# pr0g/ToyMeshPathTracer

Measured on AMD Instinct MI355X. Metric: MRays/s on sponza.obj 1920x1080 64spp at 1/2/4/8 GPUs; %HBM roofline, higher is better.
Workload: dtype f32

## Files before the change

toymeshpathtracer_amd/csrc/tmpt_api.cpp:

```cpp
#include <dlfcn.h>
#include <hip/hip_runtime.h>
#include <rccl/rccl.h>
#include <string.h>

#include <algorithm>
#include <new>
#include <chrono>
#include <string>
#include <thread>
#include <vector>

#include "tmpt.h"
#include "tmpt_internal.h"
#include "tmpt_traverse.h"
#include "tmpt_render.h"
#include "tmpt_query_key.h"

namespace tmpt {

static thread_local std::string g_last_error;
void set_error(const std::string& msg) { g_last_error = msg; }
const char* last_error() { return g_last_error.c_str(); }

int load_obj(const char* path, std::vector<float>& tris, f3& bmin, f3& bmax);
// ... 79 lines not shown
    {"sah_c_leaf", true, 0, 1e6, nullptr, &Options::sah_c_leaf, nullptr},
    {"sah_c_tri", true, 0, 1e6, nullptr, &Options::sah_c_tri, nullptr},
    {"sample_base", false, 0, 64512, &Options::sample_base, nullptr, nullptr},
    {"sample_block", false, 0, 1024, &Options::sample_block, nullptr, nullptr},
    {"sample_tail", false, -1, 64, &Options::sample_tail, nullptr, nullptr},
    {"sbuf_max", false, 0, 1e18, nullptr, nullptr, &Options::sbuf_max},
    {"sbuf_pair", false, 0, 1, &Options::sbuf_pair, nullptr, nullptr},
    {"cam_pre", false, -1, 1, &Options::cam_pre, nullptr, nullptr},
    {"cam_pre_max", false, 0, 1e18, nullptr, nullptr, &Options::cam_pre_max},
    {"shadow_split", false, 0, 1, &Options::shadow_split, nullptr, nullptr},
    {"shadow_split_max", false, 0, 1e18, nullptr, nullptr, &Options::shadow_split_max},
    {"shadow_split_pass", false, 0, 1024, &Options::shadow_split_pass, nullptr, nullptr},
    {"pilot", false, -1, 512, &Options::pilot, nullptr, nullptr},
    {"help", false, -1, 1, &Options::help, nullptr, nullptr},
    {"pair", false, -1, 63, &Options::pair, nullptr, nullptr},
    {"balance", false, 0, 1, &Options::balance, nullptr, nullptr},
    {"dprio", false, 0, 1, &Options::dprio, nullptr, nullptr},
    {"wave_cap", false, 0, 64, &Options::wave_cap, nullptr, nullptr},
    {"pixel_chains", false, -1, 1024, &Options::pixel_chains, nullptr, nullptr},
    {"tie_defer", false, -1, 1, &Options::tie_defer, nullptr, nullptr},
    {"redo_cap", false, 0, 1 << 30, &Options::redo_cap, nullptr, nullptr},
    {"redo_inline", false, 0, 1, &Options::redo_inline, nullptr, nullptr},
    {"redo_lanes", false, 1, 64, &Options::redo_lanes, nullptr, nullptr},
    {"path_waves", false, 0, 6, &Options::path_waves, nullptr, nullptr},
    {"top_walk", false, -1, 8, &Options::top_walk, nullptr, nullptr},
    {"shadow_order", false, -1, 2, &Options::shadow_order, nullptr, nullptr},
    {"pop_cull", false, -1, 1, &Options::pop_cull, nullptr, nullptr},
    {"pop_key_cap", false, -1, kPopKeyMax, &Options::pop_key_cap, nullptr, nullptr},
    {"rowspec", false, 0, 1, &Options::rowspec, nullptr, nullptr},
    {"rowspec_wmax", false, 0, 16384, &Options::rowspec_wmax, nullptr, nullptr},
    {"rowspec_windows", false, 0, 32, &Options::rowspec_windows, nullptr, nullptr},
    {"rowspec_spread", false, -1, 100, nullptr, &Options::rowspec_spread, nullptr},
    {"rowspec_groups", false, 1, kRowSpecMaxGroups, &Options::rowspec_groups, nullptr, nullptr},
    {"rowspec_noshadow", false, 0, 1, &Options::rowspec_noshadow, nullptr, nullptr},
    {"rowspec_chase", false, 0, 1, &Options::rowspec_chase, nullptr, nullptr},
    {"rowspec_stream", false, 0, 1, &Options::rowspec_stream, nullptr, nullptr},
    {"rowstream_dynamic", false, 0, 1, &Options::rowstream_dynamic, nullptr, nullptr},
    {"row_flag_leaves", false, 0, 1, &Options::row_flag_leaves, nullptr, nullptr},
    {"row_occ", false, 0, 5, &Options::row_occ, nullptr, nullptr},
    {"wf_bins", false, 1, 8, &Options::wf_bins, nullptr, nullptr},
    {"rowstream_test_abort", false, 0, 1, &Options::rowstream_test_abort, nullptr, nullptr},
    {"tie_rule", false, 0, 1, &Options::tie_rule, nullptr, nullptr},
    {"aov_group", false, 0, 16, &Options::aov_group, nullptr, nullptr},
    {"octree_build", false, 0, 1, &Options::octree_build, nullptr, nullptr},
    {"octree_dev_max", false, 0, 1e18, nullptr, nullptr, &Options::octree_dev_max},
    {"denoise_lds", false, -1, 1, &Options::denoise_lds, nullptr, nullptr},
// ... 266 lines not shown
    if (s.stream.ensure(hipStreamNonBlocking) != hipSuccess) return fail((set_error("tmpt_scene_create: no stream"), -1));
    DeviceBuffer<float> d_tris;
    if (n > 0) {
        if (!d_tris.alloc(sizeof(float) * 9 * (size_t)n))
            return fail((set_error("tmpt_scene_create: out of device memory"), -1));
        if (hipMemcpy(d_tris, tris, sizeof(float) * 9 * (size_t)n, hipMemcpyHostToDevice) != hipSuccess)
            return fail((set_error("tmpt_scene_create: upload failed"), -1));
    }
    s.tris_host.assign(tris, tris + 9 * (size_t)n);
    const int rc = build_lbvh(s.bvh, s.opt, s.stream, d_tris);
    d_tris.reset();
    if (rc) return fail(rc);
    *out = h;
    return 0;
    TMPT_GUARD_END
}

int tmpt_scene_destroy(tmpt_scene* h)
{
    if (!h) return 0;
    Scene& s = h->s;
    (void)hipSetDevice(s.device);
    if (s.stream) (void)hipStreamSynchronize(s.stream);
    for (auto& st : s.rs_stream)
        if (st) (void)hipStreamSynchronize(st);
    delete h;
    return 0;
}

int tmpt_scene_build_octree(tmpt_scene* h, const float bmin[3], const float bmax[3])
{
    TMPT_GUARD_BEGIN
    if (!h || !bmin || !bmax) return bad("tmpt_scene_build_octree: null argument");
    Scene& s = h->s;
    if ((int64_t)s.tris_host.size() != 9 * (int64_t)s.bvh.n) return bad("tmpt_scene_build_octree: no triangle copy");
    TMPT_HIP(hipSetDevice(s.device));
    const auto t0 = std::chrono::steady_clock::now();
    OctreeHost t;
    Octree o;
    const bool on_device = s.opt.octree_build == 1;
    double wmax[3] = {0.0, 0.0, 0.0};
    if (on_device) {
        (void)hipGetLastError();
        if (int rc = build_octree_device(s, bmin, bmax, o, wmax)) return rc;
    } else {
        build_octree(s.tris_host.data(), s.bvh.n, bmin, bmax, t);
// ... 243 lines not shown
    }
    return rc;
    TMPT_GUARD_END
}

int tmpt_scene_get_option(const tmpt_scene* h, const char* key, double* value)
{
    TMPT_GUARD_BEGIN
    if (!h || !value) return bad("tmpt_scene_get_option: null argument");
    if (key && strcmp(key, "pop_key_bits") == 0) {
        *value = (double)pop_key_bits(h->s.bvh.link_bits, h->s.opt.pop_key_cap);
        return 0;
    }
    if (key && strcmp(key, "cam_rays_used") == 0) {
        *value = (double)h->s.cam_rays_used;
        return 0;
    }
    if (key && strcmp(key, "shadow_split_used") == 0) {
        *value = (double)h->s.split_used;
        return 0;
    }
    if (key && strcmp(key, "path_waves_used") == 0) {
        *value = (double)h->s.path_waves_used;
        return 0;
    }
    if (key && strcmp(key, "shadow_split_resolve_ms") == 0) {
        *value = h->s.split_resolve_ms;
        return 0;
    }
    if (key && strcmp(key, "update_kind") == 0) {
        *value = (double)h->s.update_kind;
        return 0;
    }
    if (key && strcmp(key, "update_ms") == 0) {
        *value = h->s.update_ms;
        return 0;
    }
    if (key && strcmp(key, "live_device_objects") == 0) {
        *value = (double)g_live_device_objects.load();
        return 0;
    }
    if (key && strcmp(key, "query_ms") == 0) return (*value = h->s.query_ms, 0);
    if (key && strcmp(key, "query_sort_ms") == 0) return (*value = h->s.query_sort_ms, 0);
    if (key && strcmp(key, "query_chunks") == 0) return (*value = (double)h->s.query_chunks, 0);
    if (key && strcmp(key, "query_sorted") == 0) return (*value = (double)h->s.query_sorted, 0);
    if (key && strcmp(key, "bvh_cost") == 0) {
// ... 1016 lines not shown
```

toymeshpathtracer_amd/csrc/tmpt_device.h:

```cpp
#pragma once

#include <hip/hip_runtime.h>
#include <stdint.h>

#include <atomic>
#include <utility>

namespace tmpt {

inline std::atomic<int64_t> g_live_device_objects{0};

inline size_t free_budget(size_t num, size_t den, size_t already_held)
{
    size_t fr = 0, tot = 0;
    if (hipMemGetInfo(&fr, &tot) != hipSuccess) fr = 0;
    return fr / den * num + already_held;
}

template <typename T = void>
class DeviceBuffer {
public:
    DeviceBuffer() = default;
    DeviceBuffer(DeviceBuffer&& o) noexcept : p_(std::exchange(o.p_, nullptr)), bytes_(std::exchange(o.bytes_, 0)) {}
    DeviceBuffer& operator=(DeviceBuffer&& o) noexcept
// ... 111 lines not shown
    Stream(Stream&& o) noexcept : h_(std::exchange(o.h_, nullptr)) {}
    ~Stream() { reset(); }
    hipStream_t get() const { return h_; }
    operator hipStream_t() const { return h_; }
    void reset()
    {
        if (h_) {
            (void)hipStreamDestroy(h_);
            --g_live_device_objects;
        }
        h_ = nullptr;
    }
    hipError_t ensure(unsigned flags = hipStreamNonBlocking)
    {
        if (h_) return hipSuccess;
        const hipError_t e = hipStreamCreateWithFlags(&h_, flags);
        if (e != hipSuccess) {
            h_ = nullptr;
            return e;
        }
        ++g_live_device_objects;
        return hipSuccess;
    }

private:
    hipStream_t h_ = nullptr;
};

}
```

toymeshpathtracer_amd/csrc/tmpt_internal.h:

```cpp
#pragma once

#include <hip/hip_runtime.h>
#include <stdint.h>

#include <string>
#include <vector>

#include "tmpt_device.h"
#include "tmpt_math.h"

namespace tmpt {

struct alignas(16) Bvh4Node {
    float4 a;
    uint4 b;
    uint4 c;
    int4 d;
};
static_assert(sizeof(Bvh4Node) == 64, "BVH4Q node is one half cache line");

constexpr int kLeafMaxTris = 16;

constexpr int kPopKeyMin = 9;
constexpr int kPopKeyMax = 16;
// ... 195 lines not shown
    int pilot = -1;
    int help = -1;
    int pair = -1;
    int balance = 1;
    int dprio = 1;
    int wave_cap = 0;
    int pixel_chains = -1;
    int rowspec = 1;
    int rowspec_wmax = 0;
    int rowspec_windows = 0;
    float rowspec_spread = -1.0f;
    int rowspec_groups = 2;
    int rowspec_noshadow = 1;
    int rowspec_chase = 1;
    int rowspec_stream = 1;
    int rowstream_test_abort = 0;
    int wf_bins = 1;
    int tie_rule = 0;
    int tie_defer = -1;
    int redo_cap = 0;
    int redo_lanes = 4;
    int path_waves = 0;
    int redo_inline = 1;
    int top_walk = -1;
    int shadow_order = -1;
    int pop_cull = -1;
    int pop_key_cap = -1;
    int aov_group = 0;
    int motion_tile = -1;
    int octree_build = 0;
    double octree_dev_max = 0.0;
    int query_sort = -1;
    int query_top = -1;
    double query_max = 0.0;
    int query_chunk = 1 << 22;
    int query_grid = 0;
    int query_legacy = 0;
    int denoise_lds = -1;
};
int options_parse(Options& o, const char* text, bool allow_build);
int options_set(Options& o, const char* key, double value, bool allow_build);
int options_get(const Options& o, const char* key, double* value);

struct Bvh {
    int32_t n = 0;
    int32_t n_nodes = 0;
// ... 7 lines not shown
    SoaScene soa;
    std::vector<int32_t> level_begin;
    DeviceBuffer<float> node_box;
    DeviceBuffer<float> rec_box;
    double build_ms = 0.0;
};

struct Octree {
    DeviceBuffer<OctNode> oct;
    DeviceBuffer<int32_t> oct_refs;
    DeviceBuffer<OctView> oct_view;
    int32_t n_oct = 0, oct_leaves = 0, oct_depth = 0;
    int32_t oct_flat = 0;
    OctGrid oct_grid{};
    int64_t n_oct_refs = 0;
    double oct_build_ms = 0.0;
    float oct_lo[3] = {0, 0, 0}, oct_hi[3] = {0, 0, 0};
};

struct Scene {
    int device = 0;
    Stream stream;
    Stream rs_stream[kRowSpecMaxGroups];
    Bvh bvh;
    std::vector<float> tris_host;
    int32_t update_kind = 0;
    double update_ms = 0.0;
    double cost = 0.0;
    bool cost_known = false;
    Event update_ev[2];
    Octree octree;
    std::vector<DeviceBuffer<>> oct_scratch;
    DeviceBuffer<uint32_t> oct_flags;
    unsigned long long* ties = nullptr;
    uint64_t tie_queries = 0, root_misses = 0, crack_queries = 0;
    int32_t row_engine = 0, stream_fallbacks = 0;
    int64_t chain_pixels = 0;
    Options opt;
    Event wait_ev;
    DeviceBuffer<unsigned long long> counters;
    PinnedBuffer<unsigned long long> counters_host;
    DeviceBuffer<uint32_t> chk;
    Event render_ev[2];
    DeviceBuffer<> ws;
    DeviceBuffer<float> motion_prev;
    DeviceBuffer<> clip_stage;
// ... 3 lines not shown
    DeviceBuffer<uint32_t> jt;
    int32_t jt_spp = 0;
    DeviceBuffer<float4> sbuf;
    DeviceBuffer<> cam_rays;
    int32_t cam_rays_used = 0;
    DeviceBuffer<> split_buf;
    int32_t split_used = 0, split_passes = 0;
    int32_t path_waves_used = 0;
    DeviceBuffer<float4> split_carry;
    bool split_sub = false;
    struct SplitAcc {
        double extend_ms = 0.0, shadow_ms = 0.0, resolve_ms = 0.0, redo_ms = 0.0;
        int64_t redo_samples = 0, redo_late = 0;
        int32_t redo_launches = 0, launches = 0, used = 0;
    } split_acc;
    Event split_ev[3];
    double split_resolve_ms = 0.0;
    DeviceBuffer<uint2> redo;
    uint32_t redo_cap = 0;
    DeviceBuffer<float4> redo_state;
    int64_t redo_samples = 0;
    int64_t redo_late = 0;
    int32_t redo_launches = 0;
    int32_t tie_path = 0;
    bool row_render = false;
    bool pixel_render = false;
    double redo_ms = 0.0;
    uint64_t redo_rays = 0;
    DeviceBuffer<uint32_t> jt2;
    int32_t jt2_n = 0;
    DeviceBuffer<> rs_buf;
    Event rs_event[kRowSpecMaxGroups + 1];
    PinnedBuffer<uint32_t> rs_host;
    DeviceBuffer<> rs_list;
    DeviceBuffer<> rss_buf;
    DeviceBuffer<uint32_t> rss_tab;
    PinnedBuffer<uint32_t> rss_host;
    bool adapt_on = false;
    const uint32_t* adapt_list = nullptr;
    int64_t adapt_n = 0;
    DeviceBuffer<> adapt_buf;
    PinnedBuffer<uint32_t> adapt_host;
    DeviceBuffer<> query_buf;
    Event query_ev[2];
    std::vector<Event> query_sort_ev;
    double query_ms = 0.0, query_sort_ms = 0.0;
// ... 53 lines not shown
```

toymeshpathtracer_amd/csrc/tmpt_path.h:

```cpp
#pragma once

#include "tmpt_render.h"

namespace tmpt {

#ifndef TMPT_RSS_T
#define TMPT_RSS_T 8
#endif
constexpr int kRssT = TMPT_RSS_T;
static_assert(kRssT >= 4 && kRssT <= 31, "the worker's pick key holds the slot in 5 bits");
constexpr uint32_t kRssM24 = 0xFFFFFFu;
struct RsStream {
    unsigned long long* __restrict__ slots;
    unsigned long long* __restrict__ res;
    unsigned long long* __restrict__ chainpos;
    uint32_t* __restrict__ list;
    uint32_t* __restrict__ rowrays;
    uint32_t* __restrict__ lo;
    uint32_t* __restrict__ ctl;
    const uint32_t* __restrict__ anchors;
    const uint32_t* __restrict__ t1;
    const uint32_t* __restrict__ t2;
    uint32_t na, R, rmask;
    uint32_t jlimit;
// ... 124 lines not shown
constexpr int path_tail(int samp) { return samp <= 1 ? kSparse : 2; }

using PathFn = void (*)(SceneView, RenderArgs, PathCtl, uint32_t*, uint32_t*, unsigned long long*);

PathFn path_kernel(const PathVariant& v);
int find_path_kernel(const PathVariant& v, const char* who, PathFn& fn);

struct PixelChains {
    const uint32_t* cpix;
    const float4* cinit;
    int n, smp0, cspp;
};

uint32_t top_walk_cap(const Options& o, int seeding);
uint32_t oct_shadow_check(const Scene& s);

void launch_resolve_px(hipStream_t stream, const float4* sbuf, int64_t P, int32_t spp, float spp_recip,
                       uint32_t* out);

size_t shadow_ovf_words(int device);
int launch_shadow(hipStream_t stream, int device, const SceneView& sv, const uint4* sq, const uint32_t* count,
                  uint32_t cap, uint32_t* head, float4* srec, uint32_t n_rec, uint32_t* ovf);
void launch_split_resolve(hipStream_t stream, const float4* srec, int64_t P, int32_t cnt, float spp_recip,
                          uint32_t* out, const float4* carry_in = nullptr, float4* carry_out = nullptr);

#ifdef TMPT_EXP_WAVETIME
constexpr int kWaveTimeMax = 16384;
bool wavetime_get(unsigned long long* w);
bool rowtime_get(unsigned long long* r, unsigned long long* cl);
void wavetime_put(const unsigned long long* w);
void rowtime_put(const unsigned long long* r);
#endif

}
```

toymeshpathtracer_amd/csrc/tmpt_render.hip:

```cpp
#include <hip/hip_runtime.h>

#include <stdio.h>
#include <stdlib.h>
#include <string.h>

#include <algorithm>
#include <chrono>
#include <cmath>
#include <string>
#include <utility>
#include <vector>

#include "tmpt_lane_path.h"
#include "tmpt_path.h"

namespace tmpt {

#ifdef TMPT_EXP_WAVETIME
__device__ unsigned long long g_wavetime[3 * kWaveTimeMax];
__device__ unsigned long long g_rowtime[kWaveTimeMax];
__device__ unsigned long long g_claimtime[kWaveTimeMax];
bool wavetime_get(unsigned long long* w)
{
    return hipMemcpyFromSymbol(w, HIP_SYMBOL(g_wavetime), 3 * kWaveTimeMax * 8) == hipSuccess;
// ... 92 lines not shown
    const float h[8] = {o.x, o.y, o.z, __uint_as_float(rng), d.x, d.y, d.z, 0.0f};
#pragma unroll
    for (int i = 0; i < 7; ++i) __hip_atomic_store(&w[i], h[i], __ATOMIC_RELAXED, __HIP_MEMORY_SCOPE_AGENT);
    for (uint32_t i = 0; i < depth; ++i)
        __hip_atomic_store(&w[8 + i], light[i * ls], __ATOMIC_RELAXED, __HIP_MEMORY_SCOPE_AGENT);
}

__device__ __forceinline__ void split_rec_put(float4* rec, f3 end, uint32_t depth, const float* light, uint32_t ls)
{
    typedef float f32x4 __attribute__((ext_vector_type(4)));
    f32x4* q = reinterpret_cast<f32x4*>(rec);
    __builtin_nontemporal_store((f32x4){end.x, end.y, end.z, __uint_as_float(depth)}, q);
    if (depth > 0u)
        __builtin_nontemporal_store((f32x4){light[0], light[ls], light[2 * ls], light[3 * ls]}, q + 1);
    if (depth > 4u)
        __builtin_nontemporal_store((f32x4){light[4 * ls], light[5 * ls], light[6 * ls], light[7 * ls]}, q + 2);
    if (depth > 8u) __builtin_nontemporal_store((f32x4){light[8 * ls], light[9 * ls], 0.0f, 0.0f}, q + 3);
}

template <int BLOCK, int SL>
__device__ __forceinline__ void redo_sample(const SceneView& sv, const RenderArgs& a, uint32_t pix, uint32_t smp_depth,
                                            const float4* __restrict__ ps, float4* __restrict__ sbuf, uint32_t sb_ss,
                                            uint32_t sb_sp, uint32_t& rays_e, uint32_t& rays_s,
                                            TravStack<BLOCK, SL>& st, float* lbuf, float4* __restrict__ srec = nullptr)
{
    const uint32_t smp = smp_depth & 0xFFFFu, depth = smp_depth >> 16;
    const float* w = reinterpret_cast<const float*>(ps);
    float h[7];
#pragma unroll
    for (int i = 0; i < 7; ++i) h[i] = __hip_atomic_load(&w[i], __ATOMIC_RELAXED, __HIP_MEMORY_SCOPE_AGENT);
    for (uint32_t i = 0; i < depth; ++i)
        lbuf[i * BLOCK] = __hip_atomic_load(&w[8 + i], __ATOMIC_RELAXED, __HIP_MEMORY_SCOPE_AGENT);
    uint32_t rng = __float_as_uint(h[3]);
    TravCount cnt;
    if (srec) {
        int end_depth = 0;
        const f3 e = trace_path<false, BLOCK, SL, true, false>(sv, mk(h[0], h[1], h[2]), mk(h[4], h[5], h[6]), rng,
                                                               rays_e, rays_s, st, lbuf, cnt, false, (int)depth,
                                                               &end_depth);
        const uint32_t cnt_smp = (uint32_t)(a.smp_end - a.smp_begin);
        split_rec_put(srec + 4 * ((size_t)pix * cnt_smp + (smp - (uint32_t)a.smp_begin)), e, (uint32_t)end_depth, lbuf,
                      BLOCK);
        return;
    }
    const f3 c = trace_path<false, BLOCK, SL, true, false>(sv, mk(h[0], h[1], h[2]), mk(h[4], h[5], h[6]), rng, rays_e,
                                                           rays_s, st, lbuf, cnt, false, (int)depth);
    typedef float f32x4 __attribute__((ext_vector_type(4)));
    __builtin_nontemporal_store((f32x4){c.x, c.y, c.z, 0.0f},
                                reinterpret_cast<f32x4*>(sbuf + ((size_t)smp * sb_ss + (size_t)pix * sb_sp)));
}

__device__ __forceinline__ uint2 redo_load(const uint2* p)
{
    const unsigned long long w =
        __hip_atomic_load(reinterpret_cast<const unsigned long long*>(p), __ATOMIC_RELAXED, __HIP_MEMORY_SCOPE_AGENT);
    return make_uint2((uint32_t)w, (uint32_t)(w >> 32));
}

__device__ __forceinline__ void redo_put(uint2* p, uint32_t pix, uint32_t smp_depth)
{
    __hip_atomic_store(reinterpret_cast<unsigned long long*>(p), ((unsigned long long)smp_depth << 32) | pix,
                       __ATOMIC_RELAXED, __HIP_MEMORY_SCOPE_AGENT);
}

__device__ __forceinline__ void redo_mark(uint2* p)
// ... 5 lines not shown
__global__ void __launch_bounds__(BLOCK) k_redo(SceneView sv, RenderArgs a, uint2* __restrict__ list, uint32_t cap,
                                                const float4* __restrict__ state, float4* __restrict__ sbuf,
                                                uint32_t sb_ss, uint32_t sb_sp,
                                                uint32_t* __restrict__ ovf, unsigned long long* __restrict__ counters)
{
    __shared__ uint32_t s_stack[SL * BLOCK];
    __shared__ float s_light[kMaxDepth * BLOCK];
    __shared__ uint4 s_top[kTopNodes * 4];
    const int64_t gtid = (int64_t)blockIdx.x * BLOCK + threadIdx.x;
    TravStack<BLOCK, SL> st{&s_stack[threadIdx.x], ovf + gtid * (kStackTotal - SL)};
    const uint32_t ntop = (uint32_t)min(kTopNodes, sv.n_nodes4);
    const uint4* g = reinterpret_cast<const uint4*>(sv.nodes4);
    for (uint32_t i = threadIdx.x; i < ntop * 4; i += BLOCK) s_top[i] = g[i];
    __syncthreads();
    st.top = (const lds_u4*)s_top;
    st.ntop = ntop;
    const uint32_t n = (uint32_t)min(counters[kRedoCounter], (unsigned long long)cap);
    uint32_t rays_e = 0, rays_s = 0;
    for (uint32_t i = (uint32_t)gtid; i < n; i += gridDim.x * BLOCK) {
        const uint2 e = list[i];
        if (e.x >= kRedoDone) continue;
        redo_sample<BLOCK, SL>(sv, a, e.x, e.y, state + (size_t)i * kRedoState4, sbuf, sb_ss, sb_sp, rays_e, rays_s,
                               st, &s_light[threadIdx.x], SPLIT ? sbuf : nullptr);
    }
    const uint32_t re = wave_sum(rays_e), rs = wave_sum(rays_s);
    if (lane_id() == 0 && re + rs) {
        atomicAdd(&counters[0], (unsigned long long)(re + rs));
        atomicAdd(&counters[3], (unsigned long long)re);
        atomicAdd(&counters[kRedoRaysCounter], (unsigned long long)(re + rs));
    }
}

static void free_redo(Scene& s)
{
    s.redo.reset();
    s.redo_state.reset();
    s.redo_cap = 0;
}
static bool alloc_redo(Scene& s, int64_t cap)
{
    free_redo(s);
    if (!s.redo.alloc(sizeof(uint2) * (size_t)cap) ||
        !s.redo_state.alloc(sizeof(float4) * kRedoState4 * (size_t)cap)) {
        free_redo(s);
        return false;
    }
// ... 463 lines not shown
                            settled = true;
                        }
                    } while (T != 0);
                }
            }
            bool finish = false, want_off = false, emit = false;
            f3 color = mk(0.0f, 0.0f, 0.0f);
            if (has_pix && !in_query && !cam) {
                if (HELP && waiting) {
                    finish = true;
                    if (depth < (uint32_t)kMaxDepth) color = sky(r.d);
                } else if (!qany) {
                    bool drop = false;
                    if (DEFER) {
                        drop = octree_flag(sv, r, ts);
                        if (wany(drop)) {
                            if (drop) {
                                const unsigned long long slot = atomicAdd(&counters[kRedoCounter], 1ull);
                                if (slot < (unsigned long long)pc.redo_cap) {
                                    redo_state_put(pc.redo_state + (size_t)slot * kRedoState4, r.o, r.d, rng, light,
                                                   depth, LS);
                                    __builtin_amdgcn_fence(__ATOMIC_RELEASE, "agent");
                                    redo_put(pc.redo + slot, pix, smp | (depth << 16));
                                }
                                rays_e -= 1u;
                                depth = 0;
                                ts.best = -1;
                            }
                        }
                        ts.best >>= 1;
                    } else if (SAMP >= 2) {
                        const bool tie = octree_flag(sv, r, ts);
                        if (wany(tie)) {
                            if (tie) settle_closest<BLOCK, SL, true, SOA, false>(sv, r, 0.0f, kMinT, kMaxT, ts, st);
                        }
                        if (!tie) ts.best >>= 1;
                    } else if (!settled) {
                        ts.best >>= 1;
                    }
                    if (ts.best >= 0) {
                        const float4* hp = reinterpret_cast<const float4*>(sv.tri_orig + ts.best);
                        float4 ha = hp[0], hb = hp[1], hc = hp[2];
                        f3 rnd = random_unit_vector(rng);
                        materialize(ha, hb, hc);
                        const f3 nrm = mk(hc.y, hc.z, hc.w);
                        const f3 pos = hit_pos(mk(ha.x, ha.y, ha.z), mk(ha.w, hb.x, hb.y), mk(hb.z, hb.w, hc.x),
// ... 1071 lines not shown
        int64_t nb = std::min<int64_t>(P, tail_blocks * grid * kBlk);
        while (nb > 0 && (P - nb) + nb * (int64_t)blk >= (1ll << 31)) nb /= 2;
        if (nb > 0) {
            ua = (uint32_t)(P - nb);
            P = (P - nb) + nb * (int64_t)blk;
        }
    }
    int pilot = 2 * P <= 5 * (int64_t)grid * kBlk ? 2 : 4;
    if (o.pilot >= 0) pilot = o.pilot;
    const bool ordered = pilot > 0 && !count && !a.jt && a.smp_begin == 0 && a.smp_end == a.spp &&
                         a.spp >= 2 * pilot && P < (1ll << 31);
    const int64_t lanes = (int64_t)grid * kBlk;
    int help = ordered && !prof && 2 * P <= 9 * lanes ? 1 : 0;
    if (o.help >= 0) help = o.help != 0 && !count && !prof && !jt;
    const uint32_t oct_shadow = oct_shadow_check(s);
    if (oct_shadow) help = 0;
    int pair = help && ordered ? (2 * P <= 3 * lanes ? 52 : 56) : 0;
    if (o.pair >= 0) pair = o.pair;
    const bool w5 = jt ? waves5 : waves5p;
    size_t ovf_words = std::max({(size_t)grid4 * (kStackTotal - kPathSL),
                                 (size_t)std::max(grid4, grid5) * (kStackTotal - kPathSL5),
                                 (size_t)grid6 * (kStackTotal - kPathSL6)}) * kBlk;
    if (jt && o.shadow_split != 0) ovf_words = std::max(ovf_words, shadow_ovf_words(s.device));
    const size_t head_words = (size_t)kSeg * kCtr;
    const size_t hist_words = ordered ? radix_sort_hist_words((int32_t)P) : 0;
    const size_t reg_words = ordered ? 2 * (size_t)kSimdKeys + 64 + (size_t)P : 0;
    const size_t extra_words = ordered ? (size_t)P * (4 + 5) + hist_words + reg_words : 0;
    if (ensure_ws(s, (ovf_words + head_words + extra_words) * 4)) return -1;
    uint32_t* heads = s.ws.as<uint32_t>() + ovf_words;
    TMPT_HIP(hipMemsetAsync(heads, 0, head_words * 4, s.stream));
    PathCtl pc;
    memset(&pc, 0, sizeof(pc));
    pc.heads = heads;
    pc.oct_shadow = oct_shadow;
    pc.top_walk = top_walk_cap(o, a.jt ? 0 : 1);
    pc.P = P;
    pc.nblk = nblk;
    pc.blk = blk;
    pc.div_nblk = fastdiv_make(nblk);
    pc.div_blk = fastdiv_make(blk);
    pc.blk0 = blk0;
    pc.ua = ua;
    if (list) pc.order = s.adapt_list;
    RenderArgs as = a;
    if (a.jt) {
        as.bmask = nblk > 1 ? blk - 1u : 2047u;
// ... 70 lines not shown
                PathFn fn6;
                if (int rc = find_path_kernel(v6, "tmpt_render", fn6)) return rc;
                if (occupancy_blocks((const void*)fn6, kBlk, 0) >= 6) {
                    v_main = v6;
                    fn_main = fn6;
                    grid_main = occupancy_grid((const void*)fn6, kBlk, 0, s.device);
                    return 0;
                }
            }
            v_main.sl = w5 ? kPathSL5 : kPathSL;
            v_main.occ = w5 ? 5 : prof ? 1 : 4;
            if (int rc = find_path_kernel(v_main, "tmpt_render", fn_main)) return rc;
            grid_main = occupancy_grid((const void*)fn_main, kBlk, 0, s.device);
            return 0;
        };
        if (int rc = pick_main()) return rc;
        if ((size_t)grid_main * kBlk * (kStackTotal - v_main.sl) > ovf_words) {
            set_error("tmpt_render: internal: stack spill area sized for fewer lanes");
            return -1;
        }
        s.path_waves_used = v_main.occ;
        s.tie_path = !oct ? 0 : redo ? 2 : redo_nomem ? 3 : 1;
        s.path_launches = 1;
        for (int attempt = 0;; ++attempt) {
            pc.redo = redo ? s.redo : nullptr;
            pc.redo_state = redo ? s.redo_state : nullptr;
            pc.redo_cap = redo ? s.redo_cap : 0u;
            pc.redo_inline = o.redo_inline ? 1u : 0u;
            pc.redo_lanes = (uint32_t)std::max(1, std::min(64, o.redo_lanes));
            if (redo) TMPT_HIP(hipMemsetAsync(s.redo, 0xFF, sizeof(uint2) * (size_t)s.redo_cap, s.stream));
            TMPT_HIP(hipEventRecord(s.path_ev[2], s.stream));
            fn_main<<<grid_main, kBlk, 0, s.stream>>>(view(s), as, pc, d_out, s.ws.as<uint32_t>(), d_counters);
            TMPT_HIP(hipGetLastError());
            TMPT_HIP(hipEventRecord(s.path_ev[3], s.stream));
            if (!redo) break;
            TMPT_HIP(hipMemcpyAsync(s.counters_host + kRedoCounter, d_counters + kRedoCounter,
                                    4 * sizeof(unsigned long long), hipMemcpyDeviceToHost, s.stream));
            TMPT_HIP(hipStreamSynchronize(s.stream));
            const unsigned long long n = s.counters_host[kRedoCounter];
            const unsigned long long traced = s.counters_host[kRedoTraced];
            s.redo_samples = (int64_t)n;
            if (n > s.redo_cap && attempt == 0) {
                if (!(n < (1ull << 31) && alloc_redo(s, (int64_t)n))) {
                    redo = false;
                    v_main.ties = 2;
                    if (int rc = pick_main()) return rc;
                    if ((size_t)grid_main * kBlk * (kStackTotal - v_main.sl) > ovf_words) {
                        set_error("tmpt_render: internal: stack spill area sized for fewer lanes");
                        return -1;
                    }
                    s.path_waves_used = v_main.occ;
                    s.redo_samples = 0;
                    s.tie_path = 3;
                }
                TMPT_HIP(hipMemsetAsync(d_counters, 0, kRenderCounters * sizeof(unsigned long long), s.stream));
                TMPT_HIP(hipMemsetAsync(heads, 0, head_words * 4, s.stream));
                if (split_on) TMPT_HIP(hipMemsetAsync(pc.sq_ctl, 0, kSplitCtlWords * 4, s.stream));
                continue;
            }
            s.redo_late = (int64_t)(std::min<unsigned long long>(n, s.redo_cap) - std::min(traced, n));
            if (traced < std::min<unsigned long long>(n, s.redo_cap)) {
                TMPT_HIP(hipEventRecord(s.path_ev[0], s.stream));
                if (split_on)
                    k_redo<kBlk, kPathSL, true><<<grid, kBlk, 0, s.stream>>>(view(s), as, s.redo, s.redo_cap,
                                                                            s.redo_state, pc.srec, pc.sb_ss, pc.sb_sp,
                                                                            s.ws.as<uint32_t>(), d_counters);
                else
                    k_redo<kBlk, kPathSL><<<grid, kBlk, 0, s.stream>>>(view(s), as, s.redo, s.redo_cap, s.redo_state,
                                                                      pc.sbuf, pc.sb_ss, pc.sb_sp, s.ws.as<uint32_t>(),
                                                                      d_counters);
                TMPT_HIP(hipGetLastError());
                TMPT_HIP(hipEventRecord(s.path_ev[1], s.stream));
                s.redo_launches = 1;
            }
            break;
        }
        if (split_on) {
            TMPT_HIP(hipEventRecord(s.split_ev[0], s.stream));
            if (launch_shadow(s.stream, s.device, view(s), pc.sq, pc.sq_ctl, pc.sq_cap, pc.sq_ctl + kCtr, pc.srec,
                              (uint32_t)cam_n, s.ws.as<uint32_t>())) {
                set_error("tmpt_render: k_shadow launch failed");
                return -1;
            }
            TMPT_HIP(hipEventRecord(s.split_ev[1], s.stream));
            launch_split_resolve(s.stream, pc.srec, a.slots, (int32_t)(s1 - s0), a.out_recip, d_out,
                                 a.smp_begin > 0 ? a.prog : nullptr, a.prog);
            TMPT_HIP(hipGetLastError());
            TMPT_HIP(hipEventRecord(s.split_ev[2], s.stream));
            return 0;
        }
        if (pc.sbuf && !s.adapt_on) {
            k_resolve_px<<<(unsigned)((a.slots + 63) / 64), 64, 0, s.stream>>>(
                pc.sbuf, a.slots, a.spp, a.out_recip, d_out, a.smp_begin, a.smp_end, a.prog);
            TMPT_HIP(hipGetLastError());
        }
        return 0;
    }
    s.tie_path = oct ? 1 : 0;
    PathFn fn;
    if (int rc = find_path_kernel(variant(w5, help, flag ? 2 : 0, false), "tmpt_render", fn)) return rc;
    const int grid_px = occupancy_grid((const void*)fn, kBlk, 0, s.device);
    s.path_waves_used = w5 ? 5 : prof ? 1 : 4;
    if ((size_t)grid_px * kBlk * (kStackTotal - (waves5p ? kPathSL5 : kPathSL)) > ovf_words) {
        set_error("tmpt_render: internal: stack spill area sized for fewer lanes");
        return -1;
    }
    uint32_t* base = heads + head_words;
    float4* state = reinterpret_cast<float4*>(base);
    uint32_t* cost = base + 4 * (size_t)P;
    uint32_t* keys = cost + P;
    uint32_t* vals = keys + P;
    uint32_t* tkeys = vals + P;
    uint32_t* tvals = tkeys + P;
// ... 153 lines not shown
    }
    return inside ? 0 : 1;
}

void reset_render_stats(Scene& s)
{
    s.extend_ms = s.shadow_ms = 0;
    s.extend_rays = s.shadow_rays = s.node_visits = s.tri_tests = 0;
    s.shadow_node_visits = s.shadow_tri_tests = 0;
    s.extend_launches = s.shadow_launches = s.iterations = 0;
    s.row_engine = 0;
    s.stream_fallbacks = 0;
    s.chain_pixels = 0;
    s.redo_samples = 0;
    s.redo_late = 0;
    s.redo_launches = 0;
    s.redo_ms = 0.0;
    s.redo_rays = 0;
    s.tie_path = 0;
    s.cam_rays_used = 0;
    s.split_used = 0;
    s.split_passes = 0;
    s.path_waves_used = 0;
    s.split_resolve_ms = 0.0;
}

int camera_rays(Scene& s, const tmpt_camera* cam, const tmpt_render_desc* d, uint32_t* out)
{
    RenderArgs a = make_args(cam, d);
    if (int rc = ensure_sample_tables(s, a.spp, "tmpt_camera_rays")) return rc;
    a.jt = s.jt;
    a.root_check = camera_root_check(s, a.cam);
    const uint32_t cnt = (uint32_t)(a.smp_end - a.smp_begin);
    const int64_t n = a.slots * (int64_t)cnt;
    if (n <= 0) return 0;
    DeviceBuffer<CamRay> buf;
    if (!buf.alloc(sizeof(CamRay) * (size_t)n)) {
        set_error("tmpt_camera_rays: out of device memory");
        return -12;
    }
    launch_cam_rays(s, a, buf);
    hipError_t e = hipGetLastError();
    if (e == hipSuccess) e = hipStreamSynchronize(s.stream);
    if (e == hipSuccess) e = hipMemcpy(out, buf, sizeof(CamRay) * (size_t)n, hipMemcpyDeviceToHost);
    if (e != hipSuccess) {
        set_error(std::string("tmpt_camera_rays: ") + hipGetErrorString(e));
// ... 54 lines not shown
                               unsigned long long* d_counters)
{
    TMPT_ALLOC(s.split_carry.reserve(sizeof(float4) * (size_t)a.slots), "tmpt_render: the shadow split's carried sums");
    Scene::SplitAcc acc;
    int rc = 0;
    int32_t tie_path = 0, passes = 0;
    for (int32_t b = 0; b < a.spp && rc == 0; b += cs, ++passes) {
        RenderArgs ap = a;
        ap.smp_begin = b;
        ap.smp_end = std::min(b + cs, a.spp);
        ap.prog = s.split_carry;
        if (b > 0) {
            TMPT_HIP(hipMemsetAsync(d_counters + kRedoCounter, 0, 4 * sizeof(unsigned long long), s.stream));
            reset_render_stats(s);
        }
        s.split_sub = true;
        rc = render_persistent(s, ap, d_out, false, d_counters);
        s.split_sub = false;
        if (rc) break;
        TMPT_HIP(hipStreamSynchronize(s.stream));
        float k = 0.0f;
        (void)hipEventElapsedTime(&k, s.path_ev[2], s.path_ev[3]);
        acc.extend_ms += k;
        if (s.redo_launches) {
            (void)hipEventElapsedTime(&k, s.path_ev[0], s.path_ev[1]);
            acc.redo_ms += k;
        }
        if (s.split_used) {
            (void)hipEventElapsedTime(&k, s.split_ev[0], s.split_ev[1]);
            acc.shadow_ms += k;
            (void)hipEventElapsedTime(&k, s.split_ev[1], s.split_ev[2]);
            acc.resolve_ms += k;
        }
        acc.redo_samples += s.redo_samples;
        acc.redo_late += s.redo_late;
        acc.redo_launches += s.redo_launches;
        acc.launches += s.path_launches;
        acc.used += s.split_used;
        if (b == 0) tie_path = s.tie_path;
    }
    if (rc) return rc;
    s.split_acc = acc;
    s.split_passes = passes;
    s.tie_path = tie_path;
    return 0;
}

// ... 116 lines not shown
                    ml.push_back((w[3 * i + 1] - t0) * 0.01);
                    ex.push_back((w[3 * i + 2] - t0) * 0.01);
                }
            auto pct = [](std::vector<double> v, double q) {
                if (v.empty()) return 0.0;
                std::sort(v.begin(), v.end());
                return v[std::min(v.size() - 1, (size_t)(q * (v.size() - 1)))];
            };
            fprintf(stderr, "waves %zu; start us p0/p50/p100 %.0f/%.0f/%.0f; main loop end p0/p10/p50/p90/p100 "
                            "%.0f/%.0f/%.0f/%.0f/%.0f; exit p0/p50/p99/p100 %.0f/%.0f/%.0f/%.0f\n",
                    st.size(), pct(st, 0), pct(st, 0.5), pct(st, 1), pct(ml, 0), pct(ml, 0.1), pct(ml, 0.5),
                    pct(ml, 0.9), pct(ml, 1), pct(ex, 0), pct(ex, 0.5), pct(ex, 0.99), pct(ex, 1));
            std::fill(w.begin(), w.end(), 0ull);
            wavetime_put(w.data());
        }
    }
#endif
    if (progressive) s.prog_key[6] = a.smp_end < a.spp ? a.smp_end : -1;
    if (persistent) {
        float k1 = 0.0f, k0 = 0.0f;
        (void)hipEventElapsedTime(&k1, s.path_ev[2], s.path_ev[3]);
        if (s.path_launches == 2) (void)hipEventElapsedTime(&k0, s.path_ev[0], s.path_ev[1]);
        s.extend_ms = (double)k0 + (double)k1;
        if (s.redo_launches) {
            float kr = 0.0f;
            (void)hipEventElapsedTime(&kr, s.path_ev[0], s.path_ev[1]);
            s.redo_ms = kr;
            s.redo_rays = c[kRedoRaysCounter];
        }
        if (s.split_passes > 1) {
            const Scene::SplitAcc& acc = s.split_acc;
            s.extend_ms = acc.extend_ms;
            s.shadow_ms = acc.shadow_ms;
            s.split_resolve_ms = acc.resolve_ms;
            s.redo_ms = acc.redo_ms;
            s.redo_samples = acc.redo_samples;
            s.redo_late = acc.redo_late;
            s.redo_launches = acc.redo_launches;
            s.redo_rays = c[kRedoRaysCounter];
            s.path_launches = acc.launches;
            s.shadow_launches = s.split_used = acc.used;
        } else if (s.split_used) {
            float ks = 0.0f, kr = 0.0f;
            (void)hipEventElapsedTime(&ks, s.split_ev[0], s.split_ev[1]);
            (void)hipEventElapsedTime(&kr, s.split_ev[1], s.split_ev[2]);
            s.shadow_ms = ks;
            s.split_resolve_ms = kr;
// ... 88 lines not shown
```

toymeshpathtracer_amd/csrc/tmpt_shadow.hip:

```cpp
#include "tmpt_path.h"

namespace tmpt {

#ifndef TMPT_SHADOW_SL
#define TMPT_SHADOW_SL 12
#endif
#ifndef TMPT_SHADOW_OCC
#define TMPT_SHADOW_OCC 8
#endif
#ifndef TMPT_SHADOW_STEPS
#define TMPT_SHADOW_STEPS 1
#endif
#ifndef TMPT_SHADOW_FILL
#define TMPT_SHADOW_FILL 16
#endif
constexpr int kShadowSL = TMPT_SHADOW_SL;
constexpr int kShadowOcc = TMPT_SHADOW_OCC;
constexpr int kShadowSteps = TMPT_SHADOW_STEPS;
constexpr int kShadowFillMin = TMPT_SHADOW_FILL;
constexpr uint32_t kShadowFetch = 512u;

template <int BLOCK, int SL>
__global__ void __launch_bounds__(BLOCK, kShadowOcc) k_shadow(SceneView sv, const uint4* __restrict__ sq,
                                                              const uint32_t* __restrict__ count, uint32_t cap,
// ... 78 lines not shown
            if (done) {
                in_query = false;
                if (ts.best >= 0) srec[(size_t)(dst >> 4) * 16u + 4u + (dst & 15u)] = 0.0f;
            }
        }
    }
}

static int shadow_grid(int device)
{
    return occupancy_grid((const void*)k_shadow<kBlk, kShadowSL>, kBlk, 0, device);
}

size_t shadow_ovf_words(int device) { return (size_t)shadow_grid(device) * kBlk * (kStackTotal - kShadowSL); }

int launch_shadow(hipStream_t stream, int device, const SceneView& sv, const uint4* sq, const uint32_t* count,
                  uint32_t cap, uint32_t* head, float4* srec, uint32_t n_rec, uint32_t* ovf)
{
    k_shadow<kBlk, kShadowSL><<<shadow_grid(device), kBlk, 0, stream>>>(sv, sq, count, cap, head,
                                                                        reinterpret_cast<float*>(srec), n_rec, ovf);
    return hipGetLastError() == hipSuccess ? 0 : -1;
}

__global__ void __launch_bounds__(64) k_split_resolve(const float4* __restrict__ srec, int64_t P, int32_t cnt,
                                                       float spp_recip, uint32_t* __restrict__ out,
                                                       const float4* carry_in, float4* carry_out)
{
    constexpr int kC = 16;
    __shared__ float4 tile[64][kC + 1];
    const int64_t p0 = (int64_t)blockIdx.x * 64;
    const int t = threadIdx.x;
    const int np = (int)min<int64_t>(64, P - p0);
    f3 col = mk(0.0f, 0.0f, 0.0f);
    if (carry_in && t < np) {
        const float4 c = carry_in[p0 + t];
        col = mk(c.x, c.y, c.z);
    }
    for (int32_t s0 = 0; s0 < cnt; s0 += kC) {
        const int nc = min(kC, cnt - s0);
        for (int e = t; e < 64 * kC; e += 64) {
            const int i = e / kC, j = e - i * kC;
            if (i < np && j < nc) {
                typedef float f32x4 __attribute__((ext_vector_type(4)));
                const f32x4* rec =
                    reinterpret_cast<const f32x4*>(srec) + 4 * ((size_t)(p0 + i) * (size_t)cnt + (size_t)(s0 + j));
                const f32x4 h = __builtin_nontemporal_load(rec);
                const uint32_t depth = __float_as_uint(h.w);
                f32x4 c0 = {0.0f, 0.0f, 0.0f, 0.0f}, c1 = c0, c2 = c0;
                if (depth > 0u) c0 = __builtin_nontemporal_load(rec + 1);
                if (depth > 4u) c1 = __builtin_nontemporal_load(rec + 2);
                if (depth > 8u) c2 = __builtin_nontemporal_load(rec + 3);
                const float cs[kMaxDepth] = {c0.x, c0.y, c0.z, c0.w, c1.x, c1.y, c1.z, c1.w, c2.x, c2.y};
                f3 color = mk(h.x, h.y, h.z);
#pragma unroll
                for (int k = kMaxDepth - 1; k >= 0; --k)
                    if ((uint32_t)k < depth) color = backward_step(color, cs[k]);
                tile[i][j] = make_float4(color.x, color.y, color.z, 0.0f);
            }
        }
        __syncthreads();
        if (t < np)
            for (int j = 0; j < nc; ++j) col = col + mk(tile[t][j].x, tile[t][j].y, tile[t][j].z);
        __syncthreads();
    }
    if (t < np) {
        if (carry_out) carry_out[p0 + t] = make_float4(col.x, col.y, col.z, 0.0f);
        out[p0 + t] = pack_pixel(col, spp_recip);
    }
}

void launch_split_resolve(hipStream_t stream, const float4* srec, int64_t P, int32_t cnt, float spp_recip,
                          uint32_t* out, const float4* carry_in, float4* carry_out)
{
    k_split_resolve<<<(unsigned)((P + 63) / 64), 64, 0, stream>>>(srec, P, cnt, spp_recip, out, carry_in, carry_out);
}

}
```

Before: 12460.

## Run redo samples on a high-priority stream overlapping the shadow pass

Adds a k_redo_beside kernel launched on a new high-priority stream, so deferred redo path samples are traced concurrently with the shadow kernel instead of in a separate synchronized pass. Redo samples write their own split records, and the main path kernel pre-stores cosine prefixes when inline redo is disabled. The split resolve kernel moves to 256-thread blocks with unconditional record loads and a compact float LDS tile. It also bails out when the redo list overflowed, in which case the old host-side retry path still runs. This adds cross-stream dependencies and extra overflow-stack space, and the early exit risks leaving pixels unresolved in some edge cases.

```diff
diff --git a/toymeshpathtracer_amd/csrc/tmpt_api.cpp b/toymeshpathtracer_amd/csrc/tmpt_api.cpp
--- a/toymeshpathtracer_amd/csrc/tmpt_api.cpp
+++ b/toymeshpathtracer_amd/csrc/tmpt_api.cpp
@@ -125,6 +125,8 @@
     {"redo_cap", false, 0, 1 << 30, &Options::redo_cap, nullptr, nullptr},
     {"redo_inline", false, 0, 1, &Options::redo_inline, nullptr, nullptr},
     {"redo_lanes", false, 1, 64, &Options::redo_lanes, nullptr, nullptr},
+    {"redo_overlap", false, -1, 1, &Options::redo_overlap, nullptr, nullptr},
+    {"redo_overlap_lanes", false, 0, 64, &Options::redo_overlap_lanes, nullptr, nullptr},
     {"path_waves", false, 0, 6, &Options::path_waves, nullptr, nullptr},
     {"top_walk", false, -1, 8, &Options::top_walk, nullptr, nullptr},
     {"shadow_order", false, -1, 2, &Options::shadow_order, nullptr, nullptr},
@@ -437,6 +439,7 @@
     Scene& s = h->s;
     (void)hipSetDevice(s.device);
     if (s.stream) (void)hipStreamSynchronize(s.stream);
+    if (s.redo_stream) (void)hipStreamSynchronize(s.redo_stream);
     for (auto& st : s.rs_stream)
         if (st) (void)hipStreamSynchronize(st);
     delete h;
@@ -726,6 +729,10 @@
     }
     if (key && strcmp(key, "path_waves_used") == 0) {
         *value = (double)h->s.path_waves_used;
+        return 0;
+    }
+    if (key && strcmp(key, "redo_overlap_used") == 0) {
+        *value = (double)h->s.redo_overlap_used;
         return 0;
     }
     if (key && strcmp(key, "shadow_split_resolve_ms") == 0) {
diff --git a/toymeshpathtracer_amd/csrc/tmpt_device.h b/toymeshpathtracer_amd/csrc/tmpt_device.h
--- a/toymeshpathtracer_amd/csrc/tmpt_device.h
+++ b/toymeshpathtracer_amd/csrc/tmpt_device.h
@@ -157,6 +157,20 @@
         ++g_live_device_objects;
         return hipSuccess;
     }
+    hipError_t ensure_high_priority(unsigned flags = hipStreamNonBlocking)
+    {
+        if (h_) return hipSuccess;
+        int least = 0, greatest = 0;
+        hipError_t e = hipDeviceGetStreamPriorityRange(&least, &greatest);
+        if (e != hipSuccess) return e;
+        e = hipStreamCreateWithPriority(&h_, flags, greatest);
+        if (e != hipSuccess) {
+            h_ = nullptr;
+            return e;
+        }
+        ++g_live_device_objects;
+        return hipSuccess;
+    }
 
 private:
     hipStream_t h_ = nullptr;
diff --git a/toymeshpathtracer_amd/csrc/tmpt_internal.h b/toymeshpathtracer_amd/csrc/tmpt_internal.h
--- a/toymeshpathtracer_amd/csrc/tmpt_internal.h
+++ b/toymeshpathtracer_amd/csrc/tmpt_internal.h
@@ -241,6 +241,8 @@
     int redo_lanes = 4;
     int path_waves = 0;
     int redo_inline = 1;
+    int redo_overlap = -1;
+    int redo_overlap_lanes = 0;
     int top_walk = -1;
     int shadow_order = -1;
     int pop_cull = -1;
@@ -294,6 +296,7 @@
     int device = 0;
     Stream stream;
     Stream rs_stream[kRowSpecMaxGroups];
+    Stream redo_stream;
     Bvh bvh;
     std::vector<float> tris_host;
     int32_t update_kind = 0;
@@ -343,6 +346,7 @@
     int64_t redo_samples = 0;
     int64_t redo_late = 0;
     int32_t redo_launches = 0;
+    int32_t redo_overlap_used = 0;
     int32_t tie_path = 0;
     bool row_render = false;
     bool pixel_render = false;
diff --git a/toymeshpathtracer_amd/csrc/tmpt_path.h b/toymeshpathtracer_amd/csrc/tmpt_path.h
--- a/toymeshpathtracer_amd/csrc/tmpt_path.h
+++ b/toymeshpathtracer_amd/csrc/tmpt_path.h
@@ -170,7 +170,8 @@
 int launch_shadow(hipStream_t stream, int device, const SceneView& sv, const uint4* sq, const uint32_t* count,
                   uint32_t cap, uint32_t* head, float4* srec, uint32_t n_rec, uint32_t* ovf);
 void launch_split_resolve(hipStream_t stream, const float4* srec, int64_t P, int32_t cnt, float spp_recip,
-                          uint32_t* out, const float4* carry_in = nullptr, float4* carry_out = nullptr);
+                          uint32_t* out, const float4* carry_in = nullptr, float4* carry_out = nullptr,
+                          const unsigned long long* listed = nullptr, uint32_t list_cap = 0);
 
 #ifdef TMPT_EXP_WAVETIME
 constexpr int kWaveTimeMax = 16384;
diff --git a/toymeshpathtracer_amd/csrc/tmpt_render.hip b/toymeshpathtracer_amd/csrc/tmpt_render.hip
--- a/toymeshpathtracer_amd/csrc/tmpt_render.hip
+++ b/toymeshpathtracer_amd/csrc/tmpt_render.hip
@@ -138,7 +138,8 @@
 __device__ __forceinline__ void redo_sample(const SceneView& sv, const RenderArgs& a, uint32_t pix, uint32_t smp_depth,
                                             const float4* __restrict__ ps, float4* __restrict__ sbuf, uint32_t sb_ss,
                                             uint32_t sb_sp, uint32_t& rays_e, uint32_t& rays_s,
-                                            TravStack<BLOCK, SL>& st, float* lbuf, float4* __restrict__ srec = nullptr)
+                                            TravStack<BLOCK, SL>& st, float* lbuf, float4* __restrict__ srec = nullptr,
+                                            bool own = false)
 {
     const uint32_t smp = smp_depth & 0xFFFFu, depth = smp_depth >> 16;
     const float* w = reinterpret_cast<const float*>(ps);
@@ -155,8 +156,16 @@
                                                                rays_e, rays_s, st, lbuf, cnt, false, (int)depth,
                                                                &end_depth);
         const uint32_t cnt_smp = (uint32_t)(a.smp_end - a.smp_begin);
-        split_rec_put(srec + 4 * ((size_t)pix * cnt_smp + (smp - (uint32_t)a.smp_begin)), e, (uint32_t)end_depth, lbuf,
-                      BLOCK);
+        float4* rec = srec + 4 * ((size_t)pix * cnt_smp + (smp - (uint32_t)a.smp_begin));
+        if (own) {
+            typedef float f32x4 __attribute__((ext_vector_type(4)));
+            __builtin_nontemporal_store((f32x4){e.x, e.y, e.z, __uint_as_float((uint32_t)end_depth)},
+                                        reinterpret_cast<f32x4*>(rec));
+            float* cosine = reinterpret_cast<float*>(rec) + 4;
+            for (uint32_t k = depth; k < (uint32_t)end_depth; ++k) cosine[k] = lbuf[k * BLOCK];
+            return;
+        }
+        split_rec_put(rec, e, (uint32_t)end_depth, lbuf, BLOCK);
         return;
     }
     const f3 c = trace_path<false, BLOCK, SL, true, false>(sv, mk(h[0], h[1], h[2]), mk(h[4], h[5], h[6]), rng, rays_e,
@@ -208,6 +217,46 @@
         if (e.x >= kRedoDone) continue;
         redo_sample<BLOCK, SL>(sv, a, e.x, e.y, state + (size_t)i * kRedoState4, sbuf, sb_ss, sb_sp, rays_e, rays_s,
                                st, &s_light[threadIdx.x], SPLIT ? sbuf : nullptr);
+    }
+    const uint32_t re = wave_sum(rays_e), rs = wave_sum(rays_s);
+    if (lane_id() == 0 && re + rs) {
+        atomicAdd(&counters[0], (unsigned long long)(re + rs));
+        atomicAdd(&counters[3], (unsigned long long)re);
+        atomicAdd(&counters[kRedoRaysCounter], (unsigned long long)(re + rs));
+    }
+}
+
+constexpr int kRedoBesideBlocks = 1;
+constexpr int kRedoBesideLanes = 16;
+template <int BLOCK, int SL>
+__global__ void __launch_bounds__(BLOCK) k_redo_beside(SceneView sv, RenderArgs a, const uint2* __restrict__ list,
+                                                       uint32_t cap, const float4* __restrict__ state,
+                                                       float4* __restrict__ srec, uint32_t lanes,
+                                                       uint32_t* __restrict__ ovf,
+                                                       unsigned long long* __restrict__ counters)
+{
+    __shared__ uint32_t s_stack[SL * BLOCK];
+    __shared__ float s_light[kMaxDepth * BLOCK];
+    __shared__ uint4 s_top[kTopNodes * 4];
+    if ((unsigned long long)blockIdx.x * (BLOCK / 64) * lanes >= counters[kRedoCounter]) return;
+    const int64_t gtid = (int64_t)blockIdx.x * BLOCK + threadIdx.x;
+    TravStack<BLOCK, SL> st{&s_stack[threadIdx.x], ovf + gtid * (kStackTotal - SL)};
+    const uint32_t ntop = (uint32_t)min(kTopNodes, sv.n_nodes4);
+    const uint4* g = reinterpret_cast<const uint4*>(sv.nodes4);
+    for (uint32_t i = threadIdx.x; i < ntop * 4; i += BLOCK) s_top[i] = g[i];
+    __syncthreads();
+    st.top = (const lds_u4*)s_top;
+    st.ntop = ntop;
+    const uint32_t n = (uint32_t)min(counters[kRedoCounter], (unsigned long long)cap);
+    const uint32_t wave = (uint32_t)(gtid / 64), stride = gridDim.x * (BLOCK / 64) * lanes;
+    uint32_t rays_e = 0, rays_s = 0;
+    if ((uint32_t)lane_id() < lanes) {
+        for (uint64_t i = (uint64_t)wave * lanes + (uint32_t)lane_id(); i < n; i += stride) {
+            const uint2 e = list[i];
+            if (e.x >= kRedoDone) continue;
+            redo_sample<BLOCK, SL>(sv, a, e.x, e.y, state + (size_t)i * kRedoState4, nullptr, 0u, 0u, rays_e, rays_s, st,
+                                   &s_light[threadIdx.x], srec, true);
+        }
     }
     const uint32_t re = wave_sum(rays_e), rs = wave_sum(rays_s);
     if (lane_id() == 0 && re + rs) {
@@ -717,6 +766,12 @@
                                                    depth, LS);
                                     __builtin_amdgcn_fence(__ATOMIC_RELEASE, "agent");
                                     redo_put(pc.redo + slot, pix, smp | (depth << 16));
+                                    if (SPLIT && !pc.redo_inline) {
+                                        float* cosine = reinterpret_cast<float*>(
+                                                            pc.srec + 4 * ((size_t)pix * pc.cam_count +
+                                                                           (smp - (uint32_t)a.smp_begin))) + 4;
+                                        for (uint32_t i = 0; i < depth; ++i) cosine[i] = light[i * LS];
+                                    }
                                 }
                                 rays_e -= 1u;
                                 depth = 0;
@@ -1834,6 +1889,13 @@
                                  (size_t)std::max(grid4, grid5) * (kStackTotal - kPathSL5),
                                  (size_t)grid6 * (kStackTotal - kPathSL6)}) * kBlk;
     if (jt && o.shadow_split != 0) ovf_words = std::max(ovf_words, shadow_ovf_words(s.device));
+    int grid_beside = 0;
+    if (jt && o.shadow_split != 0 && o.redo_overlap != 0 && o.redo_inline != 0) {
+        const void* fn = (const void*)k_redo_beside<kBlk, kPathSL>;
+        grid_beside = kRedoBesideBlocks * (occupancy_grid(fn, kBlk, 0, s.device) / std::max(1, occupancy_blocks(fn, kBlk, 0)));
+        ovf_words = std::max(ovf_words,
+                             shadow_ovf_words(s.device) + (size_t)grid_beside * kBlk * (kStackTotal - kPathSL));
+    }
     const size_t head_words = (size_t)kSeg * kCtr;
     const size_t hist_words = ordered ? radix_sort_hist_words((int32_t)P) : 0;
     const size_t reg_words = ordered ? 2 * (size_t)kSimdKeys + 64 + (size_t)P : 0;
@@ -1950,11 +2012,30 @@
         s.path_waves_used = v_main.occ;
         s.tie_path = !oct ? 0 : redo ? 2 : redo_nomem ? 3 : 1;
         s.path_launches = 1;
+        auto split_tail = [&](bool beside) -> int {
+            TMPT_HIP(hipEventRecord(s.split_ev[0], s.stream));
+            if (launch_shadow(s.stream, s.device, view(s), pc.sq, pc.sq_ctl, pc.sq_cap, pc.sq_ctl + kCtr, pc.srec,
+                              (uint32_t)cam_n, s.ws.as<uint32_t>())) {
+                set_error("tmpt_render: k_shadow launch failed");
+                return -1;
+            }
+            TMPT_HIP(hipEventRecord(s.split_ev[1], s.stream));
+            if (beside) TMPT_HIP(hipStreamWaitEvent(s.stream, s.path_ev[1], 0));
+            launch_split_resolve(s.stream, pc.srec, a.slots, (int32_t)(s1 - s0), a.out_recip, d_out,
+                                 a.smp_begin > 0 ? a.prog : nullptr, a.prog,
+                                 beside ? d_counters + kRedoCounter : nullptr, s.redo_cap);
+            TMPT_HIP(hipGetLastError());
+            TMPT_HIP(hipEventRecord(s.split_ev[2], s.stream));
+            return 0;
+        };
+        const bool beside = split_on && redo && o.redo_inline != 0 && o.redo_overlap != 0 && grid_beside > 0;
+        if (beside) TMPT_HIP(s.redo_stream.ensure_high_priority());
+        bool tail_done = false;
         for (int attempt = 0;; ++attempt) {
             pc.redo = redo ? s.redo : nullptr;
             pc.redo_state = redo ? s.redo_state : nullptr;
             pc.redo_cap = redo ? s.redo_cap : 0u;
-            pc.redo_inline = o.redo_inline ? 1u : 0u;
+            pc.redo_inline = o.redo_inline && !(beside && redo) ? 1u : 0u;
             pc.redo_lanes = (uint32_t)std::max(1, std::min(64, o.redo_lanes));
             if (redo) TMPT_HIP(hipMemsetAsync(s.redo, 0xFF, sizeof(uint2) * (size_t)s.redo_cap, s.stream));
             TMPT_HIP(hipEventRecord(s.path_ev[2], s.stream));
@@ -1962,6 +2043,17 @@
             TMPT_HIP(hipGetLastError());
             TMPT_HIP(hipEventRecord(s.path_ev[3], s.stream));
             if (!redo) break;
+            if (beside) {
+                const uint32_t bl = (uint32_t)(o.redo_overlap_lanes > 0 ? o.redo_overlap_lanes : kRedoBesideLanes);
+                TMPT_HIP(hipStreamWaitEvent(s.redo_stream, s.path_ev[3], 0));
+                TMPT_HIP(hipEventRecord(s.path_ev[0], s.redo_stream));
+                k_redo_beside<kBlk, kPathSL><<<grid_beside, kBlk, 0, s.redo_stream>>>(
+                    view(s), as, s.redo, s.redo_cap, s.redo_state, pc.srec, bl,
+                    s.ws.as<uint32_t>() + shadow_ovf_words(s.device), d_counters);
+                TMPT_HIP(hipGetLastError());
+                TMPT_HIP(hipEventRecord(s.path_ev[1], s.redo_stream));
+                if (int rc = split_tail(true)) return rc;
+            }
             TMPT_HIP(hipMemcpyAsync(s.counters_host + kRedoCounter, d_counters + kRedoCounter,
                                     4 * sizeof(unsigned long long), hipMemcpyDeviceToHost, s.stream));
             TMPT_HIP(hipStreamSynchronize(s.stream));
@@ -1986,6 +2078,11 @@
                 if (split_on) TMPT_HIP(hipMemsetAsync(pc.sq_ctl, 0, kSplitCtlWords * 4, s.stream));
                 continue;
             }
+            if (beside) {
+                s.redo_overlap_used = 1;
+                tail_done = true;
+                break;
+            }
             s.redo_late = (int64_t)(std::min<unsigned long long>(n, s.redo_cap) - std::min(traced, n));
             if (traced < std::min<unsigned long long>(n, s.redo_cap)) {
                 TMPT_HIP(hipEventRecord(s.path_ev[0], s.stream));
@@ -2003,20 +2100,7 @@
             }
             break;
         }
-        if (split_on) {
-            TMPT_HIP(hipEventRecord(s.split_ev[0], s.stream));
-            if (launch_shadow(s.stream, s.device, view(s), pc.sq, pc.sq_ctl, pc.sq_cap, pc.sq_ctl + kCtr, pc.srec,
-                              (uint32_t)cam_n, s.ws.as<uint32_t>())) {
-                set_error("tmpt_render: k_shadow launch failed");
-                return -1;
-            }
-            TMPT_HIP(hipEventRecord(s.split_ev[1], s.stream));
-            launch_split_resolve(s.stream, pc.srec, a.slots, (int32_t)(s1 - s0), a.out_recip, d_out,
-                                 a.smp_begin > 0 ? a.prog : nullptr, a.prog);
-            TMPT_HIP(hipGetLastError());
-            TMPT_HIP(hipEventRecord(s.split_ev[2], s.stream));
-            return 0;
-        }
+        if (split_on) return tail_done ? 0 : split_tail(false);
         if (pc.sbuf && !s.adapt_on) {
             k_resolve_px<<<(unsigned)((a.slots + 63) / 64), 64, 0, s.stream>>>(
                 pc.sbuf, a.slots, a.spp, a.out_recip, d_out, a.smp_begin, a.smp_end, a.prog);
@@ -2216,6 +2300,7 @@
     s.split_used = 0;
     s.split_passes = 0;
     s.path_waves_used = 0;
+    s.redo_overlap_used = 0;
     s.split_resolve_ms = 0.0;
 }
 
@@ -2316,7 +2401,7 @@
         float k = 0.0f;
         (void)hipEventElapsedTime(&k, s.path_ev[2], s.path_ev[3]);
         acc.extend_ms += k;
-        if (s.redo_launches) {
+        if (s.redo_launches || s.redo_overlap_used) {
             (void)hipEventElapsedTime(&k, s.path_ev[0], s.path_ev[1]);
             acc.redo_ms += k;
         }
@@ -2479,7 +2564,7 @@
         (void)hipEventElapsedTime(&k1, s.path_ev[2], s.path_ev[3]);
         if (s.path_launches == 2) (void)hipEventElapsedTime(&k0, s.path_ev[0], s.path_ev[1]);
         s.extend_ms = (double)k0 + (double)k1;
-        if (s.redo_launches) {
+        if (s.redo_launches || s.redo_overlap_used) {
             float kr = 0.0f;
             (void)hipEventElapsedTime(&kr, s.path_ev[0], s.path_ev[1]);
             s.redo_ms = kr;
diff --git a/toymeshpathtracer_amd/csrc/tmpt_shadow.hip b/toymeshpathtracer_amd/csrc/tmpt_shadow.hip
--- a/toymeshpathtracer_amd/csrc/tmpt_shadow.hip
+++ b/toymeshpathtracer_amd/csrc/tmpt_shadow.hip
@@ -124,12 +124,19 @@
     return hipGetLastError() == hipSuccess ? 0 : -1;
 }
 
-__global__ void __launch_bounds__(64) k_split_resolve(const float4* __restrict__ srec, int64_t P, int32_t cnt,
-                                                       float spp_recip, uint32_t* __restrict__ out,
-                                                       const float4* carry_in, float4* carry_out)
+constexpr int kResolveBlk = 256;
+constexpr int kResolveC = 16;
+constexpr int kResolveRow = 3 * kResolveC + 1;
+
+__global__ void __launch_bounds__(kResolveBlk) k_split_resolve(const float4* __restrict__ srec, int64_t P, int32_t cnt,
+                                                                float spp_recip, uint32_t* __restrict__ out,
+                                                                const float4* carry_in, float4* carry_out,
+                                                                const unsigned long long* __restrict__ listed,
+                                                                uint32_t list_cap)
 {
-    constexpr int kC = 16;
-    __shared__ float4 tile[64][kC + 1];
+    constexpr int kC = kResolveC;
+    __shared__ float tile[64 * kResolveRow];
+    if (listed && *listed > (unsigned long long)list_cap) return;
     const int64_t p0 = (int64_t)blockIdx.x * 64;
     const int t = threadIdx.x;
     const int np = (int)min<int64_t>(64, P - p0);
@@ -140,29 +147,33 @@
     }
     for (int32_t s0 = 0; s0 < cnt; s0 += kC) {
         const int nc = min(kC, cnt - s0);
-        for (int e = t; e < 64 * kC; e += 64) {
+        for (int e = t; e < 64 * kC; e += kResolveBlk) {
             const int i = e / kC, j = e - i * kC;
             if (i < np && j < nc) {
                 typedef float f32x4 __attribute__((ext_vector_type(4)));
                 const f32x4* rec =
                     reinterpret_cast<const f32x4*>(srec) + 4 * ((size_t)(p0 + i) * (size_t)cnt + (size_t)(s0 + j));
                 const f32x4 h = __builtin_nontemporal_load(rec);
+                const f32x4 c0 = __builtin_nontemporal_load(rec + 1);
+                const f32x4 c1 = __builtin_nontemporal_load(rec + 2);
+                const f32x4 c2 = __builtin_nontemporal_load(rec + 3);
                 const uint32_t depth = __float_as_uint(h.w);
-                f32x4 c0 = {0.0f, 0.0f, 0.0f, 0.0f}, c1 = c0, c2 = c0;
-                if (depth > 0u) c0 = __builtin_nontemporal_load(rec + 1);
-                if (depth > 4u) c1 = __builtin_nontemporal_load(rec + 2);
-                if (depth > 8u) c2 = __builtin_nontemporal_load(rec + 3);
                 const float cs[kMaxDepth] = {c0.x, c0.y, c0.z, c0.w, c1.x, c1.y, c1.z, c1.w, c2.x, c2.y};
                 f3 color = mk(h.x, h.y, h.z);
 #pragma unroll
                 for (int k = kMaxDepth - 1; k >= 0; --k)
                     if ((uint32_t)k < depth) color = backward_step(color, cs[k]);
-                tile[i][j] = make_float4(color.x, color.y, color.z, 0.0f);
+                float* w = &tile[i * kResolveRow + 3 * j];
+                w[0] = color.x;
+                w[1] = color.y;
+                w[2] = color.z;
             }
         }
         __syncthreads();
-        if (t < np)
-            for (int j = 0; j < nc; ++j) col = col + mk(tile[t][j].x, tile[t][j].y, tile[t][j].z);
+        if (t < np) {
+            const float* r = &tile[t * kResolveRow];
+            for (int j = 0; j < nc; ++j) col = col + mk(r[3 * j], r[3 * j + 1], r[3 * j + 2]);
+        }
         __syncthreads();
     }
     if (t < np) {
@@ -172,9 +183,11 @@
 }
 
 void launch_split_resolve(hipStream_t stream, const float4* srec, int64_t P, int32_t cnt, float spp_recip,
-                          uint32_t* out, const float4* carry_in, float4* carry_out)
+                          uint32_t* out, const float4* carry_in, float4* carry_out, const unsigned long long* listed,
+                          uint32_t list_cap)
 {
-    k_split_resolve<<<(unsigned)((P + 63) / 64), 64, 0, stream>>>(srec, P, cnt, spp_recip, out, carry_in, carry_out);
+    k_split_resolve<<<(unsigned)((P + 63) / 64), kResolveBlk, 0, stream>>>(srec, P, cnt, spp_recip, out, carry_in,
+                                                                          carry_out, listed, list_cap);
 }
 
 }
```

After: 12410. About the same (-0.4%).
